# danshapero/sigma

Hardware: AMD Instinct MI355X
Metric: SpMV GB/s (achieved HBM) + CG iters/sec on 5-pt Laplacian, N=1e7 (higher is better)
Workload: dtype f64; 1 GPU; 5-point 2D Poisson CSR, 3162x3162 rows per GPU (rank 0: n=9998244, nnz=49978572), fp64 SpMV y=A*x; rows_per_gpu=9998244, nnz_per_gpu=49978572, parallelism=row-partition x1, matrix_resident_bytes_per_gpu=479920788, reference_layout_bytes_per_gpu=639735844, full=False

## Files before the change

sigma_amd/csrc/sgm_internal.hpp:

```cpp
#pragma once
#include <hip/hip_runtime.h>

#include <cstdarg>
#include <cstdint>
#include <cstdio>
#include <cstring>
#include <string>
#include <atomic>
#include <utility>
#include <vector>

#include "../../include/sigma_hip.h"

namespace sgm {

extern std::string g_err;
int fail(int code, const char *fmt, ...);

#define SGM_HIP(call)                                                              \
    do {                                                                           \
        hipError_t e__ = (call);                                                   \
        if (e__ != hipSuccess)                                                     \
            return sgm::fail(SGM_ERR_HIP, "%s:%d: %s -> %s", __FILE__, __LINE__,   \
                             #call, hipGetErrorString(e__));                       \
// ... 116 lines not shown

struct SliceSched { int32_t *tab = nullptr; int32_t lo = 0, hi = 0, grid = 0, iters = 0, band = 0; };

struct Part {
    MatOptions opt = g_opt.mat;
    int32_t n = 0;
    int32_t ncol_own = 0;
    int32_t n_halo = 0;
    int32_t int_lo = 0, int_hi = 0;
    int64_t nnz = 0;
    int64_t row_begin = 0;
    int32_t *rowptr = nullptr;
    int32_t *col = nullptr;
    double *val = nullptr;
    uint8_t *code = nullptr;
    int32_t *dict = nullptr;
    int32_t ndict = 0;
    int32_t dict_reach = 0;
    int32_t max_row = 0;
    double *sval = nullptr;
    uint32_t *scode = nullptr;
    int32_t *scol = nullptr;
    uint8_t *sbcode = nullptr;
    bool lean = false;
    double *sl_val = nullptr;
    int32_t *sl_col = nullptr;
    uint16_t *sl_perm = nullptr;
    int64_t *sl_off = nullptr;
    int64_t sl_total = 0;
    int32_t *sl_win0 = nullptr;
    int32_t sl_gs = 1;
    int32_t sl_span = 0;
    int32_t sw = 0;
    int32_t sched_period = 0;
    mutable SliceSched sched[3];
    mutable int nsched = 0;
    const int32_t *run_sched = nullptr;
    int32_t run_iters = 0;
    int32_t max_d = 0;
    int32_t *ecol = nullptr;
    double *eval = nullptr;
    int32_t *edeg = nullptr;
    uint8_t *ecode = nullptr;
    int32_t emdp = 0;
    int32_t *cb_perm = nullptr;
    double *cb_sval = nullptr;
    uint16_t *cb_lcol = nullptr;
    int32_t *cb_bstart = nullptr;
    uint16_t *cb_lpos = nullptr;
    void *cb_fdesc = nullptr;
    double *cb_P = nullptr;
    int32_t cb_cols = 0, cb_nb = 0, cb_R = 0, cb_ntiles = 0, cb_chunks = 0;
    int32_t cb_maxd = 0;
    int64_t cb_count = 0;
    double col_spread = -1.0;
    std::vector<HaloNbr> nbrs;
    double *xext = nullptr;
    int dot_grid_override = 0;
    int64_t xlen() const { return (int64_t)ncol_own + n_halo; }
};

}

namespace sgm { struct AlgPlan; void alg_plan_free(AlgPlan *p); void alg_plan_rows(const AlgPlan *p, int32_t out[2]); }

struct sgm_comm_s {
// ... 205 lines not shown
```

sigma_amd/csrc/sgm_layouts.hip:

```cpp
#include "sgm_spmv_select.hpp"

namespace sgm {

__global__ void k_dec1(int32_t *a, int64_t n)
{
    int64_t i = (int64_t)blockIdx.x * blockDim.x + threadIdx.x;
    const int64_t stride = (int64_t)gridDim.x * blockDim.x;
    for (; i < n; i += stride) a[i] -= 1;
}

__global__ void k_check_ptr1(const int32_t *__restrict__ ptr1, int64_t n, int64_t nnz, unsigned long long *bad)
{
    int64_t i = (int64_t)blockIdx.x * blockDim.x + threadIdx.x;
    const int64_t stride = (int64_t)gridDim.x * blockDim.x;
    for (; i <= n; i += stride) {
        const int32_t a = ptr1[i];
        bool ok = true;
        if (i == 0) ok = a == 1;
        if (i < n) ok = ok && ptr1[i + 1] >= a;
        else ok = ok && (int64_t)a - 1 == nnz;
        if (!ok) atomicMin(bad, (unsigned long long)i);
    }
}

// ... 227 lines not shown
        if (p.n > 0 && (mk_col || mk_val))
            hipLaunchKernelGGL(k_sell_unpack, dim3((unsigned)std::min<int64_t>((nch + 3) / 4, 65536)), dim3(256), 0, st, p.n,
                               (const int32_t *)p.rowptr, (const int64_t *)p.sl_off, (const uint16_t *)p.sl_perm, (const int32_t *)p.sl_col,
                               (const double *)p.sl_val, mk_col ? p.col : nullptr, mk_val ? p.val : nullptr);
        SGM_HIP(hipGetLastError());
        SGM_HIP(hipStreamSynchronize(st));
        return SGM_OK;
    }
    if (mk_code) { SGM_TRY(dalloc(&p.code, (size_t)nnz + 32)); SGM_HIP(hipMemsetAsync(p.code + nnz, 0, 32, st)); }
    if (p.n > 0)
        hipLaunchKernelGGL(k_sl_unpack, dim3((unsigned)std::min<int64_t>(((int64_t)p.n + 255) / 256, 4096)), dim3(256), 0, st, p.n, p.sw,
                           (const int32_t *)p.rowptr, (const uint32_t *)p.scode, (const int32_t *)p.dict, (const double *)p.sval,
                           mk_col ? p.col : nullptr, mk_val ? p.val : nullptr, mk_code ? p.code : nullptr);
    SGM_HIP(hipGetLastError());
    SGM_HIP(hipStreamSynchronize(st));
    return SGM_OK;
}
int lean_val_buffer(Part &p)
{
    if (!p.lean || p.val) return SGM_OK;
    SGM_TRY(dalloc(&p.val, (size_t)p.nnz + 2));
    SGM_HIP(hipMemsetAsync(p.val + p.nnz, 0, 2 * sizeof(double), g_rt.stream));
    return SGM_OK;
}
void csr_release_arrays(const Part &cp)
{
    Part &p = const_cast<Part &>(cp);
    if (!p.lean || !lean_applies(p)) return;
    (void)hipStreamSynchronize(g_rt.stream);
    dfree(p.val); dfree(p.col); dfree(p.code);
    p.val = nullptr; p.col = nullptr; p.code = nullptr;
}

int pack_sliced(Part &p)
{
    if (p.sl_val && p.n > 0) {
        const int64_t nch = (((int64_t)p.n + kSlRows - 1) / kSlRows) * (kSlRows / kSellChunk);
        hipLaunchKernelGGL(k_sell_fill, dim3((unsigned)std::min<int64_t>((nch + 3) / 4, 65536)), dim3(256), 0, g_rt.stream, p.n,
                           (const int32_t *)p.rowptr, (const int32_t *)nullptr, (const double *)p.val, (const int64_t *)p.sl_off,
                           (const uint16_t *)p.sl_perm, (int32_t *)nullptr, p.sl_val);
        SGM_HIP(hipGetLastError());
    }
    if ((!p.scode && !p.scol && !p.sbcode) || p.n == 0) return SGM_OK;
    const int64_t nsl = ((int64_t)p.n + kSlRows - 1) / kSlRows;
    if (p.ecol)
        hipLaunchKernelGGL(k_sl_pack_ell, dim3((unsigned)std::min<int64_t>(nsl, 65536)), dim3(256), 0, g_rt.stream, p.n, p.sw,
                           p.max_d, (const double *)p.eval, p.sval);
    else
        hipLaunchKernelGGL(k_sl_pack, dim3((unsigned)std::min<int64_t>(nsl, 65536)), dim3(256), 0, g_rt.stream, p.n, p.sw,
                           (const int32_t *)p.rowptr, (const double *)p.val, p.sval);
    SGM_HIP(hipGetLastError());
    return SGM_OK;
}

__global__ void k_fill32(int64_t n, int32_t *a, int32_t v)
{
    int64_t i = (int64_t)blockIdx.x * blockDim.x + threadIdx.x;
    const int64_t stride = (int64_t)gridDim.x * blockDim.x;
    for (; i < n; i += stride) a[i] = v;
}

constexpr int kDictSlots = 1024;
constexpr int32_t kDictEmpty = INT32_MIN;
__global__ __launch_bounds__(256) void k_dict_collect(int32_t n, const int32_t *__restrict__ rowptr, const int32_t *__restrict__ col,
                                                      int32_t *table, int *count, int *max_row)
{
    constexpr int kLocal = 512;
    __shared__ int32_t ltab[kLocal];
    __shared__ int lcount;
    for (int t = threadIdx.x; t < kLocal; t += 256) ltab[t] = kDictEmpty;
    if (threadIdx.x == 0) lcount = 0;
    __syncthreads();
    int mr = 0;
    int32_t mine[8];
#pragma unroll
    for (int t = 0; t < 8; ++t) mine[t] = kDictEmpty;
    int next = 0;
    for (int32_t i = blockIdx.x * blockDim.x + threadIdx.x; i < n; i += gridDim.x * blockDim.x) {
        const int32_t s0 = rowptr[i], e = rowptr[i + 1];
        mr = max(mr, e - s0);
        for (int32_t k = s0; k < e; ++k) {
            const int32_t off = col[k] - i;
            bool known = false;
#pragma unroll
            for (int t = 0; t < 8; ++t) known = known || mine[t] == off;
// ... 445 lines not shown
    *out = nullptr;
    if (!A || A->fmt != SGM_FMT_CSR || A->parts.size() != 1 || A->comm)
        return fail(SGM_ERR_UNSUPPORTED, "clone_csr_plain: single-GPU CSR matrices only");
    const Part &p = A->parts[0];
    SGM_TRY(csr_need_arrays(p));
    struct Release { const Part &p; ~Release() { csr_release_arrays(p); } } rel{p};
    sgm_mat C = new sgm_mat_s;
    C->fmt = SGM_FMT_CSR; C->nrow = A->nrow; C->ncol = A->ncol; C->nnz = A->nnz;
    C->parts.resize(1);
    Part &q = C->parts[0];
    q.opt.csr_offset_dict = 0; q.opt.csr_sliced = 0; q.opt.csr_sell = 0; q.opt.csr_lean = 0; q.opt.slice_sched = 0;
    q.n = p.n; q.ncol_own = p.ncol_own; q.n_halo = 0; q.nnz = p.nnz; q.max_row = p.max_row;
    hipStream_t st = g_rt.stream;
    int rc = dalloc(&q.rowptr, (size_t)p.n + 1);
    if (rc == SGM_OK) rc = dalloc(&q.col, (size_t)p.nnz + 4);
    if (rc == SGM_OK) rc = dalloc(&q.val, (size_t)p.nnz + 2);
    if (rc != SGM_OK) { sgm_mat_destroy(C); return rc; }
    (void)hipMemcpyAsync(q.rowptr, p.rowptr, ((size_t)p.n + 1) * 4, hipMemcpyDeviceToDevice, st);
    (void)hipMemsetAsync(q.col + p.nnz, 0, 16, st);
    (void)hipMemsetAsync(q.val + p.nnz, 0, 16, st);
    if (p.nnz) {
        (void)hipMemcpyAsync(q.col, p.col, (size_t)p.nnz * 4, hipMemcpyDeviceToDevice, st);
        (void)hipMemcpyAsync(q.val, p.val, (size_t)p.nnz * 8, hipMemcpyDeviceToDevice, st);
    }
    if (hipStreamSynchronize(st) != hipSuccess || hipGetLastError() != hipSuccess) { sgm_mat_destroy(C); return fail(SGM_ERR_HIP, "clone_csr_plain: copy failed"); }
    *out = C;
    return SGM_OK;
}

int rebuild_csr_formats(Part &p)
{
    SGM_TRY(csr_need_arrays(p));
    p.lean = false;
    dfree(p.code); dfree(p.dict); dfree(p.sval); dfree(p.scode); dfree(p.scol); dfree(p.sbcode);
    p.code = nullptr; p.dict = nullptr; p.sval = nullptr; p.scode = nullptr; p.scol = nullptr; p.sbcode = nullptr;
    free_sell(p);
    free_ell_colblock(p);
    p.ndict = 0; p.dict_reach = 0; p.sw = 0; p.max_row = 0; p.sched_period = 0;
    free_slice_sched(p);
    return build_offset_dict(p, nullptr, nullptr);
}
int rebuild_ell_formats(Part &p)
{
    dfree(p.ecode); dfree(p.dict); dfree(p.sval); dfree(p.scode);
    p.ecode = nullptr; p.dict = nullptr; p.dict_reach = 0; p.emdp = 0; p.sval = nullptr; p.scode = nullptr; p.sw = 0; p.sched_period = 0;
    free_slice_sched(p);
    SGM_TRY(build_ell_offset_dict(p));
    SGM_TRY(build_ell_colblock(p));
    return refresh_ell_colblock_values(p);
}
int sgm_invalidate_transpose(sgm_mat A)
{
    if (A->T) { sgm_mat_destroy(A->T); A->T = nullptr; }
    dfree(A->tperm);
    A->tperm = nullptr;
    A->t_stale = true;
    return SGM_OK;
}

void free_part(Part &p)
{
    dfree(p.rowptr); dfree(p.col); dfree(p.val); dfree(p.code); dfree(p.dict); dfree(p.sval); dfree(p.scode); dfree(p.scol); dfree(p.sbcode); dfree(p.ecol); dfree(p.eval); dfree(p.edeg); dfree(p.ecode); dfree(p.xext);
    for (auto &nb : p.nbrs) { dfree(nb.send_idx); dfree(nb.send_buf); }
    free_slice_sched(p);
    free_ell_colblock(p);
    free_sell(p);
    p = Part();
}

}
```

sigma_amd/csrc/sgm_mat.hip:

```cpp
#include "sgm_spmv_select.hpp"

namespace sgm {

struct Staged {
    double *dev = nullptr;
    bool owned = false;
    ~Staged() { if (owned) dfree(dev); }
};
int stage_in(Staged &s, const double *v, int64_t n, int where, bool copy)
{
    if (where == SGM_DEVICE && (reinterpret_cast<uintptr_t>(v) & 15) == 0) {
        s.dev = const_cast<double *>(v);
        return SGM_OK;
    }
    SGM_TRY(dalloc(&s.dev, (size_t)n));
    s.owned = true;
    if (copy)
        SGM_HIP(hipMemcpyAsync(s.dev, v, (size_t)n * 8,
                               where == SGM_HOST ? hipMemcpyHostToDevice : hipMemcpyDeviceToDevice,
                               g_rt.stream));
    return SGM_OK;
}
int stage_out(const Staged &s, double *v, int64_t n, int where)
{
// ... 361 lines not shown
    return SGM_OK;
}

int sgm_mat_set_option(sgm_mat A, const char *name, int value)
{
    SGM_TRY(require_init());
    if (!A || !name) return fail(SGM_ERR_BAD_ARG, "sgm_mat_set_option: null argument");
    int v = 0;
    SGM_TRY(normalise_option(name, value, &v));
    MatOptions probe;
    if (!mat_option_field(probe, name)) return fail(SGM_ERR_BAD_ARG, "sgm_mat_set_option: '%s' is not a matrix option", name);
    if (A->fmt == SGM_FMT_COMPOSITE) {
        for (sgm_mat_s *B : A->blocks)
            if (B) SGM_TRY(sgm_mat_set_option(B, name, value));
        return SGM_OK;
    }
    const bool cb_shape = !strcmp(name, "ell_colblock_cols") || !strcmp(name, "ell_colblock_rows");
    for (Part &p : A->parts) {
        int *f = mat_option_field(p.opt, name);
        const int old = *f;
        *f = v;
        if (old == v) continue;
        if ((p.ecol || (!p.lean && p.rowptr && p.col && p.val && p.n_halo == 0 && !p.sval && !p.sl_val)) &&
            (cb_shape || (!strcmp(name, "ell_colblock") && ((old != 0) != (v != 0) || v == 2 || old == 2)))) {
            SGM_TRY(build_ell_colblock(p));
            SGM_TRY(refresh_ell_colblock_values(p));
            SGM_HIP(hipStreamSynchronize(g_rt.stream));
        }
        if (!strcmp(name, "csr_lean") && !p.ecol) {
            if (v == 0) { SGM_TRY(csr_need_arrays(p)); p.lean = false; }
            else csr_go_lean(p);
        }
        if (!strcmp(name, "slice_sched")) free_slice_sched(p);
    }
    if (A->T) SGM_TRY(sgm_mat_set_option(A->T, name, value));
    return SGM_OK;
}

int sgm_mat_matvec(sgm_mat A, const double *x, double *y, int where)
{
    return matvec_impl(A, x, y, where, false);
}

int sgm_mat_matvec_add(sgm_mat A, const double *x, double *y, int where)
{
    return matvec_impl(A, x, y, where, true);
}

int sgm_composite_create(sgm_mat *out, int32_t nrb, int32_t ncb, const int32_t *row_ptr, const int32_t *col_ptr,
                         const sgm_mat *blocks)
{
    SGM_TRY(require_init());
    if (!out || nrb < 1 || ncb < 1 || !row_ptr || !col_ptr || !blocks)
        return fail(SGM_ERR_BAD_ARG, "sgm_composite_create: bad argument");
    sgm_mat A = new sgm_mat_s;
    A->fmt = SGM_FMT_COMPOSITE;
    for (int i = 0; i <= nrb; ++i) A->blk_row_ptr.push_back(row_ptr[i] - 1);
    for (int j = 0; j <= ncb; ++j) A->blk_col_ptr.push_back(col_ptr[j] - 1);
    A->nrow = A->blk_row_ptr[nrb];
    A->ncol = A->blk_col_ptr[ncb];
    A->blocks.assign(blocks, blocks + (size_t)nrb * ncb);
    sgm_comm comm = nullptr;
    bool any_local = false;
    for (int it = 0; it < nrb; ++it)
        for (int jt = 0; jt < ncb; ++jt) {
            sgm_mat C = A->blocks[(size_t)it * ncb + jt];
// ... 140 lines not shown
    else if (use_slicedb(p)) snprintf(name, len, "k_csr_slb<W=%d>", p.sw);
    else if (use_sliced32(p)) snprintf(name, len, "k_csr_sl32<W=%d>", p.sw);
    else if (use_sell(p)) snprintf(name, len, p.sl_win0 && p.opt.csr_xwindow ? "k_csr_sell<pad=%.3f,xw=%dx%d>" : "k_csr_sell<pad=%.3f>",
                                   p.nnz ? (double)p.sl_total / (double)p.nnz : 1.0, p.sl_span, p.sl_gs);
    else if (use_offset_dict(p)) snprintf(name, len, "k_csr_do<256,%d,CW=1>", do_tile_for(p));
    else if (use_row_owner(p)) snprintf(name, len, "k_csr_do<256,%d,CW=4>", do_tile_for(p));
    else if (use_row_lines(p)) snprintf(name, len, "k_csr_rl");
    else snprintf(name, len, "k_csr_spmv");
}
}
extern "C" {

int sgm_mat_kernel(sgm_mat A, char *buf, int len)
{
    if (!A || !buf || len < 1) return fail(SGM_ERR_BAD_ARG, "sgm_mat_kernel: bad argument");
    char name[64];
    if (A->fmt == SGM_FMT_COMPOSITE) snprintf(name, sizeof name, "composite");
    else part_kernel_name(A->parts[0], A->fmt, name, sizeof name);
    snprintf(buf, (size_t)len, "%s", name);
    return SGM_OK;
}

static int64_t part_resident_bytes(const Part &p)
{
    int64_t b = 0;
    const int64_t nsl = ((int64_t)p.n + kSlRows - 1) / kSlRows;
    if (p.rowptr) b += 4 * ((int64_t)p.n + 1);
    if (p.col) b += 4 * (p.nnz + 4);
    if (p.val) b += 8 * (p.nnz + 2);
    if (p.code) b += p.nnz + 16;
    if (p.dict) b += 4 * 256;
    if (p.sval) b += 8 * nsl * kSlRows * p.sw;
    if (p.scode) b += 4 * nsl * kSlRows;
    if (p.scol) b += 4 * nsl * kSlRows * p.sw;
    if (p.sbcode) b += nsl * kSlRows * ((p.sw + 7) / 8 * 8);
    if (p.sl_val) b += 12 * p.sl_total + 2 * nsl * kSlRows + 8 * (nsl * (kSlRows / kSellChunk) + 1);
    if (p.ecol) b += 4 * (int64_t)p.n * p.max_d;
    if (p.eval) b += 8 * (int64_t)p.n * p.max_d;
    if (p.edeg) b += 4 * (int64_t)p.n;
    if (p.ecode) b += (int64_t)p.n * p.emdp;
    if (p.xext) b += 8 * p.xlen();
    b += ell_colblock_resident_bytes(p);
    for (const auto &nb : p.nbrs) b += (int64_t)nb.send_count * (nb.send_buf ? 12 : 4);
    return b;
}
static int64_t part_matvec_bytes(const sgm_mat_s *A, const Part &p)
{
    const int64_t nsl = ((int64_t)p.n + kSlRows - 1) / kSlRows;
    int64_t m;
    if (A->fmt == SGM_FMT_ELL) {
        if (use_ell_colblock(p)) return ell_colblock_matvec_bytes(p);
        if (use_sliced_ell(p)) m = nsl * kSlRows * (8 * (int64_t)p.sw + 4);
        else if (p.ecode && p.opt.ell_offset_dict) m = (int64_t)p.n * (8 * (int64_t)p.max_d + p.emdp);
        else m = 12 * (int64_t)p.n * p.max_d;
    } else if (use_ell_colblock(p)) return ell_colblock_matvec_bytes(p);
    else if (use_sliced(p)) m = nsl * kSlRows * (8 * (int64_t)p.sw + 4);
    else if (use_slicedb(p)) m = nsl * kSlRows * (8 * (int64_t)p.sw + (p.sw + 7) / 8 * 8);
    else if (use_sliced32(p)) m = nsl * kSlRows * 12 * (int64_t)p.sw;
    else if (use_sell(p)) {
        m = 12 * p.sl_total + 2 * nsl * kSlRows + 8 * nsl * (kSlRows / kSellChunk);
        if (p.sl_win0 && p.opt.csr_xwindow)
            return m + ((nsl + p.sl_gs - 1) / p.sl_gs) * (8 * (int64_t)p.sl_span + 4) + 8 * (int64_t)p.n;
    }
    else if (use_offset_dict(p)) m = 9 * p.nnz + 4 * ((int64_t)p.n + 1);
    else m = 12 * p.nnz + 4 * ((int64_t)p.n + 1);
    return m + 8 * p.xlen() + 8 * (int64_t)p.n;
}

int sgm_mat_footprint(sgm_mat A, int64_t *resident_bytes, int64_t *matvec_bytes)
{
    if (!A) return fail(SGM_ERR_BAD_ARG, "sgm_mat_footprint: null matrix");
    int64_t res = 0, mv = 0;
    if (A->fmt == SGM_FMT_COMPOSITE) {
        for (sgm_mat C : A->blocks) {
            if (!C) continue;
            int64_t r = 0, m = 0;
            SGM_TRY(sgm_mat_footprint(C, &r, &m));
            mv += m + 8 * (int64_t)C->nrow;
        }
        mv += 8 * (int64_t)A->nrow;
    } else {
        for (const Part &p : A->parts) { res += part_resident_bytes(p); mv += part_matvec_bytes(A, p); }
        if (A->T) { int64_t r = 0; SGM_TRY(sgm_mat_footprint(A->T, &r, nullptr)); res += r + 4 * A->nnz; }
    }
    if (resident_bytes) *resident_bytes = res;
    if (matvec_bytes) *matvec_bytes = mv;
    return SGM_OK;
}

// ... 13 lines not shown
```

sigma_amd/csrc/sgm_runtime.hip:

```cpp
#include "sgm_internal.hpp"

#include <algorithm>

namespace sgm {

std::string g_err;
Runtime g_rt;
Options g_opt;
Heartbeat g_hb;
extern int g_force_collectives;

int fail(int code, const char *fmt, ...)
{
    char buf[1024];
    va_list ap;
    va_start(ap, fmt);
    vsnprintf(buf, sizeof buf, fmt, ap);
    va_end(ap);
    g_err = buf;
    return code;
}

bool trace_on()
{
// ... 60 lines not shown
    SGM_HIP(hipStreamSynchronize(st));
    return SGM_OK;
}

#define SGM_OPT(group, field) if (!strcmp(name, #field)) return &o.field;
int *mat_option_field(MatOptions &o, const char *name)
{
    SGM_OPT(mat, csr_offset_dict) SGM_OPT(mat, ell_offset_dict) SGM_OPT(mat, csr_row_owner) SGM_OPT(mat, csr_row_lines)
    SGM_OPT(mat, csr_sliced) SGM_OPT(mat, csr_sell) SGM_OPT(mat, csr_xwindow) SGM_OPT(mat, csr_lean) SGM_OPT(mat, ell_colblock) SGM_OPT(mat, ell_colblock_cols)
    SGM_OPT(mat, ell_colblock_rows) SGM_OPT(mat, slice_sched) SGM_OPT(mat, coloring_pass)
    return nullptr;
}
int *solver_option_field(SolverOptions &o, const char *name)
{
    SGM_OPT(solver, cg_small) SGM_OPT(solver, bicgstab_small) SGM_OPT(solver, krylov_graph) SGM_OPT(solver, dot_order)
    SGM_OPT(solver, gmres_cgs2) SGM_OPT(solver, dist_halo_fused) SGM_OPT(solver, coop_spin_limit) SGM_OPT(solver, cg_coop_variant)
    SGM_OPT(solver, reorder_solve)
    return nullptr;
}
int *pc_option_field(PcOptions &o, const char *name)
{
    SGM_OPT(pc, ildu_strips) SGM_OPT(pc, ildu_rows) SGM_OPT(pc, pipeline_spin_limit) SGM_OPT(pc, ildu_reorder)
    return nullptr;
}
#undef SGM_OPT

int normalise_option(const char *name, int value, int *out)
{
    int v = value;
    if (!strcmp(name, "ell_colblock_cols")) v = std::min(kEllcbMaxCols, std::max(2, value)) & ~1;
    else if (!strcmp(name, "ell_colblock_rows")) v = value == 512 ? 512 : value == 256 ? 256 : 0;
    else if (!strcmp(name, "ildu_reorder")) v = value != 0;
    else if (!strcmp(name, "csr_sell")) v = value < 0 ? 0 : value > 2 ? 2 : value;
    else if (!strcmp(name, "csr_lean") || !strcmp(name, "csr_xwindow")) v = value != 0;
    else if (!strcmp(name, "slice_sched")) v = value <= 0 ? 0 : value == 1 ? 1 : std::max(4, value);
    else if (!strcmp(name, "krylov_graph")) v = value <= 0 ? 0 : value == 1 ? 1 : std::max(16, (value + 15) / 16 * 16);
    else if (!strcmp(name, "cg_small")) v = std::max(0, value);
    else if (!strcmp(name, "dist_halo_fused") || !strcmp(name, "reorder_solve")) v = value < 0 ? 0 : value > 2 ? 2 : value;
    else if (!strcmp(name, "coop_spin_limit")) v = std::max(0, value);
    else if (!strcmp(name, "gmres_cgs2")) v = value != 0;
    else if (!strcmp(name, "cg_coop_variant")) {
        const int r = value & 15;
        if (value < 0 || value > 31 || (r != 0 && r != 1 && r != 2 && r != 4 && r != 8))
            return fail(SGM_ERR_BAD_ARG, "option cg_coop_variant: rows per thread 0 (by size), 1, 2, 4 or 8, + 16 = no one-XCD variant");
    }
    else if (!strcmp(name, "coloring_pass")) v = value < 0 ? 0 : value > 2 ? 2 : value;
    else if (!strcmp(name, "pipeline_spin_limit")) v = std::max(0, value);
    else if (!strcmp(name, "dot_order") && value != 0 && value != 1)
        return fail(SGM_ERR_BAD_ARG, "option dot_order is 0 (tree) or 1 (the reference's sequential order)");
    *out = v;
    return SGM_OK;
}

}

using namespace sgm;

extern "C" {

int sgm_init(int device)
{
    int count = 0;
    hipError_t e = hipGetDeviceCount(&count);
    if (e != hipSuccess || count <= 0)
        return fail(SGM_ERR_NO_DEVICE,
                    "sgm_init: no HIP device visible (%s); this library has no CPU path",
// ... 110 lines not shown
```

sigma_amd/csrc/sgm_spmv.hip:

```cpp
#include "sgm_spmv_select.hpp"
#include "sgm_plan_host.hpp"

namespace sgm {




__device__ inline int64_t rowblock_of(int it, int b, int grid, int64_t nrb = 0, int mode = 1)
{
    const int per = grid >> 3;
    if (mode == 2) {
        const int64_t chunk = (nrb + 7) / 8;
        const int64_t local = (int64_t)it * per + (b >> 3);
        return local < chunk ? (int64_t)(b & 7) * chunk + local : nrb;
    }
    return (int64_t)it * grid + (int64_t)(b & 7) * per + (b >> 3);
}


template <class T>
__device__ inline T ld_stream(const T *p, bool nt)
{
    return nt ? __builtin_nontemporal_load(p) : *p;
}
// ... 319 lines not shown
            while (k < kend) {
                const int cnt = min(kend - k, U);
                double xv[U], vv[U];
#pragma unroll
                for (int u = 0; u < U; ++u)
                    if (u < cnt) {
                        const int o = k + u - ts;
                        xv[u] = CW == 1 ? x[row + dl[cl[o]]] : x[(int32_t)cl4[o]];
                        vv[u] = vl[o];
                    }
#pragma unroll
                for (int u = 0; u < U; ++u)
                    if (u < cnt) z = z + vv[u] * xv[u];
                k += cnt;
            }
        }
        if (row < n) {
            const double yi = ADD ? (chain ? z : y0 + z) : 0.0 + z;
            __builtin_nontemporal_store(yi, y + row);
            if (DOT_W) dwy += w[row] * yi;
            if (DOT_YY) dyy += yi * yi;
        }
    }
    if (DOT_W) {
        const double t = block_sum<BLOCK>(dwy, red);
        if (tid == 0) part_wy[blockIdx.x] = t;
    }
    if (DOT_YY) {
        const double t = block_sum<BLOCK>(dyy, red);
        if (tid == 0) part_yy[blockIdx.x] = t;
    }
}

template <int W, bool ADD, bool DOT_W, bool DOT_YY>
__global__ __launch_bounds__(256) void k_csr_sl(
    int32_t n, const uint32_t *__restrict__ scode, const int32_t *__restrict__ dict,
    const double *__restrict__ sval, const double *__restrict__ x, double *__restrict__ y,
    const double *__restrict__ w, double *__restrict__ part_wy, double *__restrict__ part_yy,
    const int *__restrict__ flag_done, int gen, int remap, const int32_t *__restrict__ sched, int sched_iters)
{
    constexpr int BLOCK = 256;
    __shared__ int32_t dl[16];
    __shared__ double red[BLOCK / 64];
    const int st = flag_done ? *flag_done : 0;
    const int tid = threadIdx.x;
    const bool chain = (remap & 256) != 0;
    const int32_t dv = tid < 16 ? dict[tid] : 0;
    const int64_t nsl = ((int64_t)n + kSlRows - 1) / kSlRows;
    double dwy = 0.0, dyy = 0.0;

    int64_t first = blockIdx.x;
    if ((remap & 255) >= 3) {
        const int G = (remap & 255) == 3 ? 8 : (remap & 255) == 4 ? 2 : (remap & 255) == 6 ? 64 : (remap & 255) == 7 ? 128 : 32;
        const int xcd = blockIdx.x & 7, loc = blockIdx.x >> 3;
        first = (int64_t)(loc / G) * (8 * G) + xcd * G + loc % G;
    }
    int64_t sl = sched ? sched[blockIdx.x] : first;
    int sit = 0;
    u32x2 cw = {0xffffffffu, 0xffffffffu};
    f64x2 v[W];
    auto load_slice = [&](int64_t s_) {
        const int32_t row_ = (int32_t)(s_ * kSlRows) + 2 * tid;
        cw = __builtin_nontemporal_load(reinterpret_cast<const u32x2 *>(scode + row_));
        const f64x2 *vb = reinterpret_cast<const f64x2 *>(sval + s_ * (int64_t)(W * kSlRows)) + tid;
#pragma unroll
        for (int u = 0; u < W; ++u) v[u] = __builtin_nontemporal_load(vb + u * BLOCK);
    };
    bool have = sl >= 0 && sl < nsl;
    if (have) load_slice(sl);
    if (st && gen >= st) return;
    if (tid < 16) dl[tid] = dv;
    __syncthreads();
    while (have) {
        int64_t nxt = sl + gridDim.x;
        if (sched) { ++sit; nxt = sit < sched_iters ? sched[(int64_t)sit * gridDim.x + blockIdx.x] : -1; }
        const int32_t row = (int32_t)(sl * kSlRows) + 2 * tid;
        f64x2 y0 = {0.0, 0.0};
        if (ADD) {
            if (row + 1 < n) y0 = *reinterpret_cast<const f64x2 *>(y + row);
            else if (row < n) y0.x = y[row];
        }
        double xa[W], xb[W];
#pragma unroll
        for (int u = 0; u < W; ++u) {
            const uint32_t ca = (cw.x >> (4 * u)) & 15u, cb = (cw.y >> (4 * u)) & 15u;
            xa[u] = ca != 15u ? x[row + dl[ca]] : 0.0;
            xb[u] = cb != 15u ? x[row + 1 + dl[cb]] : 0.0;
        }
        f64x2 z;
        z.x = (ADD && chain) ? y0.x : 0.0;
        z.y = (ADD && chain) ? y0.y : 0.0;
#pragma unroll
        for (int u = 0; u < W; ++u) {
            if (((cw.x >> (4 * u)) & 15u) != 15u) z.x = z.x + v[u].x * xa[u];
            if (((cw.y >> (4 * u)) & 15u) != 15u) z.y = z.y + v[u].y * xb[u];
        }
        f64x2 yi;
        yi.x = ADD ? (chain ? z.x : y0.x + z.x) : 0.0 + z.x;
        yi.y = ADD ? (chain ? z.y : y0.y + z.y) : 0.0 + z.y;
        if (row + 1 < n) {
            __builtin_nontemporal_store(yi, reinterpret_cast<f64x2 *>(y + row));
            if (DOT_W) { const f64x2 wv = *reinterpret_cast<const f64x2 *>(w + row); dwy += wv.x * yi.x; dwy += wv.y * yi.y; }
            if (DOT_YY) { dyy += yi.x * yi.x; dyy += yi.y * yi.y; }
        } else if (row < n) {
            __builtin_nontemporal_store(yi.x, y + row);
            if (DOT_W) dwy += w[row] * yi.x;
            if (DOT_YY) dyy += yi.x * yi.x;
        }
        sl = nxt;
        have = sl >= 0 && sl < nsl;
        if (have) load_slice(sl);
    }
    if (DOT_W) {
        const double t = block_sum<BLOCK>(dwy, red);
        if (tid == 0) part_wy[blockIdx.x] = t;
    }
    if (DOT_YY) {
        const double t = block_sum<BLOCK>(dyy, red);
        if (tid == 0) part_yy[blockIdx.x] = t;
    }
}

template <bool ADD, bool DOT_W, bool DOT_YY, bool XW = false, int GS = 1>
__global__ __launch_bounds__(256 * GS) void k_csr_sell(
    int32_t n, const int64_t *__restrict__ off, const uint16_t *__restrict__ perm, const int32_t *__restrict__ scol,
    const double *__restrict__ sval, const double *__restrict__ x, double *__restrict__ y, const double *__restrict__ w,
    double *__restrict__ part_wy, double *__restrict__ part_yy, const int *__restrict__ flag_done, int gen, int remap,
    const int32_t *__restrict__ win0 = nullptr, int32_t span = 0, int32_t xlen = 0)
// ... 448 lines not shown
    const int tile = do_tile_for(p);
    const bool dict = use_offset_dict(p);
#define L(B, T, DW, DY)                                                                                 \
    do {                                                                                                \
        if (dict)                                                                                       \
            hipLaunchKernelGGL((k_csr_do<B, T, 1, ADD, DW, DY>), dim3(grid), dim3(B), 0, st, p.n, p.rowptr, \
                               p.code, p.dict, p.val, x, y, w, pwy, pyy, flag, gen, c.remap | g_launch_flags); \
        else                                                                                            \
            hipLaunchKernelGGL((k_csr_do<B, T, 4, ADD, DW, DY>), dim3(grid), dim3(B), 0, st, p.n, p.rowptr, \
                               reinterpret_cast<const uint8_t *>(p.col), p.dict, p.val, x, y, w, pwy, pyy, flag, \
                               gen, c.remap | g_launch_flags);                                          \
    } while (0)
#define LV(B, T)                                \
    if (c.block == B && tile == T) {            \
        if (w && pyy) L(B, T, true, true);      \
        else if (w) L(B, T, true, false);       \
        else if (pyy) L(B, T, false, true);     \
        else L(B, T, false, false);             \
        return;                                 \
    }
    SGM_DO_VARIANTS(LV)
#undef LV
#undef L
}

template <bool ADD>
static void launch_csr_sl(const Part &p, int grid, const double *x, double *y, const double *w,
                          double *pwy, double *pyy, const int *flag, int gen)
{
    const SpmvCfg &c = spmv_cfg();
    hipStream_t st = g_rt.stream;
    int mode = c.remap == 1 ? ((grid <= kMaxGrid / 2 || (int64_t)p.n < (int64_t)32768 * kSlRows) ? 5 : 0) : (c.remap >= 3 ? c.remap : 0);
    if (mode >= 3 && grid % (8 * (mode == 3 ? 8 : mode == 4 ? 2 : mode == 6 ? 64 : mode == 7 ? 128 : 32)) != 0) mode = 0;
#define L(WW, DW, DY)                                                                                   \
    hipLaunchKernelGGL((k_csr_sl<WW, ADD, DW, DY>), dim3(grid), dim3(256), 0, st, p.n, p.scode, p.dict, \
                       p.sval, x, y, w, pwy, pyy, flag, gen, mode | g_launch_flags, p.run_sched, p.run_iters)
#define LV(WW)                                \
    if (p.sw == WW) {                         \
        if (w && pyy) L(WW, true, true);      \
        else if (w) L(WW, true, false);       \
        else if (pyy) L(WW, false, true);     \
        else L(WW, false, false);             \
        return;                               \
    }
    SGM_SL_WIDTHS(LV)
#undef LV
#undef L
}

template <bool ADD>
static void launch_csr_sl32(const Part &p, int grid, const double *x, double *y, const double *w,
                            double *pwy, double *pyy, const int *flag, int gen)
{
    hipStream_t st = g_rt.stream;
    const SpmvCfg &c = spmv_cfg();
    int mode = c.remap == 1 ? ((grid <= kMaxGrid / 2 || (int64_t)p.n < (int64_t)32768 * kSlRows) ? 5 : 0) : (c.remap >= 3 ? c.remap : 0);
    if (mode >= 3 && grid % (8 * (mode == 3 ? 8 : mode == 4 ? 2 : mode == 6 ? 64 : mode == 7 ? 128 : 32)) != 0) mode = 0;
#define L(WW, DW, DY)                                                                                     \
    hipLaunchKernelGGL((k_csr_sl32<WW, ADD, DW, DY>), dim3(grid), dim3(256), 0, st, p.n, p.scol, p.sval, x, y, \
                       w, pwy, pyy, flag, gen, mode | g_launch_flags)
#define LV(WW)                                \
    if (p.sw == WW) {                         \
        if (w && pyy) L(WW, true, true);      \
        else if (w) L(WW, true, false);       \
        else if (pyy) L(WW, false, true);     \
        else L(WW, false, false);             \
        return;                               \
    }
    SGM_SL32_WIDTHS(LV)
#undef LV
#undef L
}

template <bool ADD>
static void launch_csr_sell(const Part &p, int grid, const double *x, double *y, const double *w,
                            double *pwy, double *pyy, const int *flag, int gen)
{
    hipStream_t st = g_rt.stream;
    const SpmvCfg &c = spmv_cfg();
// ... 57 lines not shown
static EllCfg &ell_cfg()
{
    static EllCfg c;
    static bool init = false;
    if (!init) {
        init = true;
        if (c.grid > kMaxGrid) c.grid = kMaxGrid;
    }
    return c;
}
int ell_grid(const Part &p)
{
    if (use_ell_colblock(p)) return ell_colblock_grid(p);
    if (use_sliced_ell(p)) {
        const int64_t nsl = ((int64_t)p.n + kSlRows - 1) / kSlRows;
        return (int)std::max<int64_t>(1, std::min<int64_t>(nsl, nsl >= 32768 ? kMaxGrid : kMaxGrid / 2));
    }
    int64_t g = ((int64_t)p.n + kBlock - 1) / kBlock;
    int64_t cap = ell_cfg().grid;
    if (p.ecode && p.opt.ell_offset_dict && p.emdp == 16) cap = std::min<int64_t>(cap, (int64_t)5 * g_rt.num_cu);
    return (int)std::max<int64_t>(1, std::min<int64_t>(g, cap));
}

template <bool ADD>
static void launch_ell(const Part &p, int grid, const double *x, double *y, const double *w,
                       double *pwy, double *pyy, const int *flag, int gen)
{
    if (use_ell_colblock(p)) {
        (void)launch_ell_colblock(p, grid, x, y, ADD, (g_launch_flags & 256) != 0, w, pwy, pyy, flag, gen);
        return;
    }
    if (use_sliced_ell(p)) {
        Part v;
        v.n = p.n; v.scode = p.scode; v.dict = p.dict; v.sval = p.sval; v.sw = p.sw;
        if (const SliceSched *ss = slice_sched(p, 0, p.n, grid)) { v.run_sched = ss->tab; v.run_iters = ss->iters; }
        launch_csr_sl<ADD>(v, grid, x, y, w, pwy, pyy, flag, gen);
        return;
    }
    hipStream_t st = g_rt.stream;
    const EllCfg &c = ell_cfg();
    if (p.ecode && p.opt.ell_offset_dict) {
#define LD(M, DW, DY)                                                                                   \
    hipLaunchKernelGGL((k_ell_do<M, ADD, DW, DY>), dim3(grid), dim3(kBlock), 0, st, p.n, p.max_d, p.ecode, \
                       p.dict, p.eval, x, y, w, pwy, pyy, flag, gen, g_launch_flags & 256)
#define LDV(M)                                   \
    {                                            \
        if (w && pyy) LD(M, true, true);         \
        else if (w) LD(M, true, false);          \
        else if (pyy) LD(M, false, true);        \
        else LD(M, false, false);                \
    }
        if (p.emdp == 4) LDV(4) else if (p.emdp == 8) LDV(8) else LDV(16)
#undef LDV
#undef LD
        return;
    }
#define L(UU, NTT, DW, DY)                                                                          \
    hipLaunchKernelGGL((k_ell_spmv<UU, NTT, ADD, DW, DY>), dim3(grid), dim3(kBlock), 0, st, p.n,     \
                       p.max_d, p.ecol, p.eval, x, y, w, pwy, pyy, flag, gen, g_launch_flags & 256)
#define LV(UU, NTT)                              \
    {                                            \
        if (w && pyy) L(UU, NTT, true, true);    \
        else if (w) L(UU, NTT, true, false);     \
        else if (pyy) L(UU, NTT, false, true);   \
        else L(UU, NTT, false, false);           \
    }
    if (c.u >= 16) { if (c.nt) LV(16, true) else LV(16, false) }
// ... 43 lines not shown
    for (int i = 0; i < p.nsched; ++i)
        if (p.sched[i].lo == lo && p.sched[i].hi == hi && p.sched[i].grid == grid) return p.sched[i].tab ? &p.sched[i] : nullptr;
    if (p.nsched >= 3) return nullptr;
    SliceSched &ss = p.sched[p.nsched++];
    ss.lo = lo; ss.hi = hi; ss.grid = grid; ss.tab = nullptr; ss.band = band;
    std::vector<int32_t> tab;
    int iters = 0;
    slice_sched_table(nsl, p.sched_period, grid, band, tab, iters);
    int32_t *d = nullptr;
    if (dalloc(&d, tab.size()) != SGM_OK) return nullptr;
    if (hipMemcpy(d, tab.data(), tab.size() * sizeof(int32_t), hipMemcpyHostToDevice) != hipSuccess) { dfree(d); return nullptr; }
    ss.tab = d; ss.iters = iters;
    return &ss;
}
void free_slice_sched(Part &p)
{
    for (int i = 0; i < p.nsched; ++i) { dfree(p.sched[i].tab); p.sched[i] = SliceSched(); }
    p.nsched = 0;
}

static void launch_range(sgm_mat A, const Part &p, const RowRange &r, const double *x, double *y, bool add,
                         const double *w, double *pwy, double *pyy, const int *flag_done, int gen)
{
    Part v;
    v.opt = p.opt;
    v.n = r.hi - r.lo;
    v.nnz = (int64_t)((double)p.nnz * v.n / (p.n > 0 ? p.n : 1));
    v.n_halo = p.n_halo; v.ncol_own = p.ncol_own;
    v.rowptr = p.rowptr + r.lo; v.col = p.col; v.val = p.val; v.code = p.code; v.dict = p.dict;
    v.max_row = p.max_row;
    const bool sliced = use_sliced(p), slicedb = !sliced && use_slicedb(p), sliced32 = !sliced && !slicedb && use_sliced32(p);
    if (sliced || slicedb)
        if (const SliceSched *ss = slice_sched(p, r.lo, r.hi, r.grid)) { v.run_sched = ss->tab; v.run_iters = ss->iters; }
    if (sliced) { v.sval = p.sval + (int64_t)r.lo * p.sw; v.scode = p.scode + r.lo; v.sw = p.sw; }
    if (slicedb) { v.sval = p.sval + (int64_t)r.lo * p.sw; v.sbcode = p.sbcode + (int64_t)r.lo * ((p.sw + 7) / 8 * 8); v.sw = p.sw; }
    if (sliced32) { v.sval = p.sval + (int64_t)r.lo * p.sw; v.scol = p.scol + (int64_t)r.lo * p.sw; v.sw = p.sw; }
    const bool sell = !sliced && !slicedb && !sliced32 && use_sell(p);
    if (sell) {
        v.sl_val = p.sl_val; v.sl_col = p.sl_col;
        v.sl_off = p.sl_off + r.lo / kSellChunk; v.sl_perm = p.sl_perm + r.lo;
        v.sl_gs = p.sl_gs;
        v.sl_win0 = p.sl_win0 ? p.sl_win0 + r.lo / (kSlRows * p.sl_gs) : nullptr; v.sl_span = p.sl_span;
    }
    const bool dict = use_offset_dict(p);
    const double *xs = dict ? x + r.lo : x;
    double *ys = y + r.lo;
    const double *ws = w ? w + r.lo : nullptr;
    double *pw = pwy ? pwy + r.part_off : nullptr, *py = pyy ? pyy + r.part_off : nullptr;
    if (sliced) {
        if (add) launch_csr_sl<true>(v, r.grid, xs, ys, ws, pw, py, flag_done, gen);
        else launch_csr_sl<false>(v, r.grid, xs, ys, ws, pw, py, flag_done, gen);
    } else if (slicedb) {
        if (add) launch_csr_slb<true>(v, r.grid, xs, ys, ws, pw, py, flag_done, gen);
        else launch_csr_slb<false>(v, r.grid, xs, ys, ws, pw, py, flag_done, gen);
    } else if (sliced32) {
        if (add) launch_csr_sl32<true>(v, r.grid, x, ys, ws, pw, py, flag_done, gen);
        else launch_csr_sl32<false>(v, r.grid, x, ys, ws, pw, py, flag_done, gen);
    } else if (sell) {
        if (add) launch_csr_sell<true>(v, r.grid, x, ys, ws, pw, py, flag_done, gen);
        else launch_csr_sell<false>(v, r.grid, x, ys, ws, pw, py, flag_done, gen);
    } else if (use_row_owner(p)) {
        if (add) launch_csr_do<true>(v, r.grid, xs, ys, ws, pw, py, flag_done, gen);
        else launch_csr_do<false>(v, r.grid, xs, ys, ws, pw, py, flag_done, gen);
    } else if (use_row_lines(p)) {
        if (add) launch_csr_rl<true>(v, r.grid, xs, ys, ws, pw, py, flag_done, gen);
        else launch_csr_rl<false>(v, r.grid, xs, ys, ws, pw, py, flag_done, gen);
    } else {
// ... 153 lines not shown
```

sigma_amd/csrc/sgm_spmv_select.hpp:

```cpp
#pragma once
#include "sgm_internal.hpp"

#include <type_traits>

#include <hipcub/hipcub.hpp>

#include <algorithm>
#include <cstdlib>
#include <string>
#include <vector>

namespace sgm {

typedef double f64x2 __attribute__((ext_vector_type(2)));
typedef int i32x2 __attribute__((ext_vector_type(2)));
typedef int i32x4 __attribute__((ext_vector_type(4)));
typedef uint32_t u32x2 __attribute__((ext_vector_type(2)));
typedef uint16_t u16x2 __attribute__((ext_vector_type(2)));
typedef unsigned int u32x4s __attribute__((ext_vector_type(4)));
#define SGM_SLB_WIDTHS(X) X(9) X(12) X(15) X(16) X(19) X(20) X(24) X(25) X(27) X(28) X(32)
#define SGM_SL_WIDTHS(X) X(3) X(5) X(7) X(8)
#define SGM_SL32_WIDTHS(X) X(3) X(5) X(7) X(8) X(12) X(16) X(20) X(24) X(28) X(32)
constexpr int kSlRows = 512;
constexpr int kSellChunk = 128;
constexpr int kSellSigma = 512;
static bool lean_sliced(const Part &p) { return p.scode && p.sval && p.dict && !p.ecol && !p.scol && !p.sbcode && p.sw <= 8; }
static bool lean_sell(const Part &p) { return p.sl_val && p.sl_col && !p.scode && !p.scol && !p.sbcode && !p.ecol; }
static bool lean_applies(const Part &p) { return p.opt.csr_lean && (lean_sliced(p) || lean_sell(p)); }


struct SpmvCfg { int block = 256, vpt = 2, nt = 1, maxgrid = 0, remap = 1, do_vpt = 0; };
static SpmvCfg &spmv_cfg()
{
    static SpmvCfg c;
    static bool init = false;
    if (!init) {
        init = true;
        if (c.maxgrid > kMaxGrid) c.maxgrid = kMaxGrid;
        if (c.block != 256 && c.block != 512 && c.block != 1024) c.block = 256;
        if (c.vpt != 2 && c.vpt != 4 && c.vpt != 8) c.vpt = 2;
        if (c.block == 1024 && c.vpt == 8) c.vpt = 4;
    }
    return c;
}

int resident_per_cu(bool dict, int block, int v, int cw = 4);
static const SliceSched *slice_sched(const Part &p, int32_t lo, int32_t hi, int grid);
void free_slice_sched(Part &p);
int ell_grid(const Part &p);
bool use_ell_colblock(const Part &p);
int ell_colblock_grid(const Part &p);
int build_ell_colblock(Part &p);
int refresh_ell_colblock_values(Part &p);
void free_ell_colblock(Part &p);
int launch_ell_colblock(const Part &p, int grid, const double *x, double *y, bool add, bool chain, const double *w,
                        double *pwy, double *pyy, const int *flag, int gen);
int64_t ell_colblock_resident_bytes(const Part &p);
// ... 49 lines not shown
    return (int)g;
}

struct RowRange { int32_t lo, hi; int grid, part_off; };
static int spmv_ranges(const Part &p, RowRange out[3], bool dots = true, bool whole = false)
{
    int nr = 0, off = 0;
    auto add = [&](int32_t lo, int32_t hi) {
        if (hi <= lo) return;
        out[nr] = RowRange{lo, hi, grid_for_rows(p, hi - lo, nr == 0 ? kMaxGrid / 4 : kMaxGrid / 8), off};
        off += out[nr].grid;
        ++nr;
    };
    if (p.n_halo == 0 || p.int_hi <= p.int_lo || whole) {
        if (any_sliced(p)) {
            out[0] = RowRange{0, p.n, grid_for_rows(p, p.n > 0 ? p.n : 1, kMaxGrid, dots), 0};
            return 1;
        }
        add(0, p.n > 0 ? p.n : 1);
        if (nr) out[0].hi = p.n;
        return nr;
    }
    add(p.int_lo, p.int_hi);
    add(0, p.int_lo);
    add(p.int_hi, p.n);
    return nr;
}


void free_part(Part &p);
void csr_go_lean(Part &p);
int lean_val_buffer(Part &p);
int pack_sliced(Part &p);
int build_ell_offset_dict(Part &p);
__global__ void k_ell_transpose(const int32_t *__restrict__ node, const double *__restrict__ val, int32_t *__restrict__ ecol,
                                double *__restrict__ eval, int32_t n, int32_t max_d, int32_t ncol = 0, unsigned long long *bad = nullptr);
}
```

Baseline: 6367 GB/s.

## Replace per-nonzero values with a per-code value table when codes map uniquely

After packing the sliced CSR format, a scan kernel checks whether every offset code always carries the same bit-exact value. If so, it builds a 16-entry value table, and the sliced SpMV kernel reads coefficients from shared memory instead of streaming sval. Where two adjacent rows share a code, the kernel also loads the pair of x values with one vector load. This removes most of the matrix value traffic for stencil-like matrices. The cost is an extra setup scan with a host synchronisation, a new template variant, and a much smaller modelled byte count per matvec.

```diff
diff --git a/sigma_amd/csrc/sgm_internal.hpp b/sigma_amd/csrc/sgm_internal.hpp
--- a/sigma_amd/csrc/sgm_internal.hpp
+++ b/sigma_amd/csrc/sgm_internal.hpp
@@ -172,6 +172,7 @@
     int32_t sl_gs = 1;
     int32_t sl_span = 0;
     int32_t sw = 0;
+    double *vtab = nullptr;
     int32_t sched_period = 0;
     mutable SliceSched sched[3];
     mutable int nsched = 0;
diff --git a/sigma_amd/csrc/sgm_layouts.hip b/sigma_amd/csrc/sgm_layouts.hip
--- a/sigma_amd/csrc/sgm_layouts.hip
+++ b/sigma_amd/csrc/sgm_layouts.hip
@@ -283,6 +283,78 @@
     p.val = nullptr; p.col = nullptr; p.code = nullptr;
 }
 
+__global__ __launch_bounds__(256) void k_sl_vtab_scan(int32_t n, int32_t W, const uint32_t *__restrict__ scode,
+                                                      const double *__restrict__ sval, unsigned long long *__restrict__ acc)
+{
+    __shared__ unsigned long long sand[16], sor[16];
+    __shared__ unsigned int sused;
+    if (threadIdx.x < 16) { sand[threadIdx.x] = ~0ull; sor[threadIdx.x] = 0ull; }
+    if (threadIdx.x == 0) sused = 0u;
+    __syncthreads();
+    unsigned int used = 0u;
+    const int64_t nsl = ((int64_t)n + kSlRows - 1) / kSlRows;
+    for (int64_t sl = blockIdx.x; sl < nsl; sl += gridDim.x)
+        for (int r = threadIdx.x; r < kSlRows; r += blockDim.x) {
+            const int64_t row = sl * kSlRows + r;
+            if (row >= n) break;
+            const uint32_t cw = scode[row];
+            const double *src = sval + sl * (int64_t)W * kSlRows + r;
+            for (int u = 0; u < W; ++u) {
+                const uint32_t c = (cw >> (4 * u)) & 15u;
+                if (c == 15u) continue;
+                const unsigned long long b = (unsigned long long)__double_as_longlong(src[(int64_t)u * kSlRows]);
+                atomicAnd(&sand[c], b);
+                atomicOr(&sor[c], b);
+                used |= 1u << c;
+            }
+        }
+    atomicOr(&sused, used);
+    __syncthreads();
+    const int t = threadIdx.x;
+    if (t < 16 && ((sused >> t) & 1u)) { atomicAnd(&acc[t], sand[t]); atomicOr(&acc[16 + t], sor[t]); }
+    if (t == 0 && sused) atomicOr(&acc[32], (unsigned long long)sused);
+}
+
+int find_value_table(Part &p)
+{
+    const int mode = p.opt.csr_sliced;
+    const bool want = p.scode && p.sval && !p.scol && !p.sbcode && !p.cb_sval && p.sw <= 8 && p.n > 0 && mode != 3 &&
+                      (mode == 2 || p.n >= (1 << 21));
+    if (!want) {
+        if (p.vtab) { SGM_HIP(hipStreamSynchronize(g_rt.stream)); dfree(p.vtab); p.vtab = nullptr; }
+        return SGM_OK;
+    }
+    double *buf = p.vtab;
+    p.vtab = nullptr;
+    if (!buf) SGM_TRY(dalloc(&buf, kVtabWords));
+    unsigned long long *acc = reinterpret_cast<unsigned long long *>(buf + 16);
+    SGM_HIP(hipMemsetAsync(acc, 0xff, 16 * 8, g_rt.stream));
+    SGM_HIP(hipMemsetAsync(acc + 16, 0, 17 * 8, g_rt.stream));
+    const int64_t nsl = ((int64_t)p.n + kSlRows - 1) / kSlRows;
+    hipLaunchKernelGGL(k_sl_vtab_scan, dim3((unsigned)std::min<int64_t>(nsl, 2048)), dim3(256), 0, g_rt.stream, p.n, p.sw,
+                       (const uint32_t *)p.scode, (const double *)p.sval, acc);
+    SGM_HIP(hipGetLastError());
+    unsigned long long h[33];
+    SGM_HIP(hipMemcpyAsync(h, acc, sizeof h, hipMemcpyDeviceToHost, g_rt.stream));
+    SGM_HIP(hipStreamSynchronize(g_rt.stream));
+    const uint32_t used = (uint32_t)h[32];
+    bool ok = used != 0;
+    unsigned long long tab[16] = {};
+    for (int c = 0; c < 15 && ok; ++c)
+        if ((used >> c) & 1u) { ok = h[c] == h[16 + c]; tab[c] = h[c]; }
+    if (ok) {
+        SGM_HIP(hipMemcpyAsync(buf, tab, sizeof tab, hipMemcpyHostToDevice, g_rt.stream));
+        SGM_HIP(hipStreamSynchronize(g_rt.stream));
+        p.vtab = buf;
+    } else {
+        dfree(buf);
+    }
+    if (trace_on())
+        fprintf(stderr, "[sgm] value table: %d rows, W=%d, %d codes used: %s\n", p.n, p.sw, __builtin_popcount(used),
+                ok ? "on (k_csr_sl reads no values)" : "off (a code carries more than one value)");
+    return SGM_OK;
+}
+
 int pack_sliced(Part &p)
 {
     if (p.sl_val && p.n > 0) {
@@ -301,7 +373,7 @@
         hipLaunchKernelGGL(k_sl_pack, dim3((unsigned)std::min<int64_t>(nsl, 65536)), dim3(256), 0, g_rt.stream, p.n, p.sw,
                            (const int32_t *)p.rowptr, (const double *)p.val, p.sval);
     SGM_HIP(hipGetLastError());
-    return SGM_OK;
+    return p.scode ? find_value_table(p) : SGM_OK;
 }
 
 __global__ void k_fill32(int64_t n, int32_t *a, int32_t v)
@@ -813,8 +885,8 @@
 {
     SGM_TRY(csr_need_arrays(p));
     p.lean = false;
-    dfree(p.code); dfree(p.dict); dfree(p.sval); dfree(p.scode); dfree(p.scol); dfree(p.sbcode);
-    p.code = nullptr; p.dict = nullptr; p.sval = nullptr; p.scode = nullptr; p.scol = nullptr; p.sbcode = nullptr;
+    dfree(p.code); dfree(p.dict); dfree(p.sval); dfree(p.scode); dfree(p.scol); dfree(p.sbcode); dfree(p.vtab);
+    p.code = nullptr; p.dict = nullptr; p.sval = nullptr; p.scode = nullptr; p.scol = nullptr; p.sbcode = nullptr; p.vtab = nullptr;
     free_sell(p);
     free_ell_colblock(p);
     p.ndict = 0; p.dict_reach = 0; p.sw = 0; p.max_row = 0; p.sched_period = 0;
@@ -823,8 +895,8 @@
 }
 int rebuild_ell_formats(Part &p)
 {
-    dfree(p.ecode); dfree(p.dict); dfree(p.sval); dfree(p.scode);
-    p.ecode = nullptr; p.dict = nullptr; p.dict_reach = 0; p.emdp = 0; p.sval = nullptr; p.scode = nullptr; p.sw = 0; p.sched_period = 0;
+    dfree(p.ecode); dfree(p.dict); dfree(p.sval); dfree(p.scode); dfree(p.vtab);
+    p.ecode = nullptr; p.dict = nullptr; p.dict_reach = 0; p.emdp = 0; p.sval = nullptr; p.scode = nullptr; p.vtab = nullptr; p.sw = 0; p.sched_period = 0;
     free_slice_sched(p);
     SGM_TRY(build_ell_offset_dict(p));
     SGM_TRY(build_ell_colblock(p));
@@ -841,7 +913,7 @@
 
 void free_part(Part &p)
 {
-    dfree(p.rowptr); dfree(p.col); dfree(p.val); dfree(p.code); dfree(p.dict); dfree(p.sval); dfree(p.scode); dfree(p.scol); dfree(p.sbcode); dfree(p.ecol); dfree(p.eval); dfree(p.edeg); dfree(p.ecode); dfree(p.xext);
+    dfree(p.rowptr); dfree(p.col); dfree(p.val); dfree(p.code); dfree(p.dict); dfree(p.sval); dfree(p.scode); dfree(p.scol); dfree(p.sbcode); dfree(p.ecol); dfree(p.eval); dfree(p.edeg); dfree(p.ecode); dfree(p.xext); dfree(p.vtab);
     for (auto &nb : p.nbrs) { dfree(nb.send_idx); dfree(nb.send_buf); }
     free_slice_sched(p);
     free_ell_colblock(p);
diff --git a/sigma_amd/csrc/sgm_mat.hip b/sigma_amd/csrc/sgm_mat.hip
--- a/sigma_amd/csrc/sgm_mat.hip
+++ b/sigma_amd/csrc/sgm_mat.hip
@@ -417,6 +417,7 @@
             else csr_go_lean(p);
         }
         if (!strcmp(name, "slice_sched")) free_slice_sched(p);
+        if (!strcmp(name, "csr_sliced") && p.scode) SGM_TRY(find_value_table(p));
     }
     if (A->T) SGM_TRY(sgm_mat_set_option(A->T, name, value));
     return SGM_OK;
@@ -623,6 +624,7 @@
     if (p.dict) b += 4 * 256;
     if (p.sval) b += 8 * nsl * kSlRows * p.sw;
     if (p.scode) b += 4 * nsl * kSlRows;
+    if (p.vtab) b += 8 * kVtabWords;
     if (p.scol) b += 4 * nsl * kSlRows * p.sw;
     if (p.sbcode) b += nsl * kSlRows * ((p.sw + 7) / 8 * 8);
     if (p.sl_val) b += 12 * p.sl_total + 2 * nsl * kSlRows + 8 * (nsl * (kSlRows / kSellChunk) + 1);
@@ -641,11 +643,11 @@
     int64_t m;
     if (A->fmt == SGM_FMT_ELL) {
         if (use_ell_colblock(p)) return ell_colblock_matvec_bytes(p);
-        if (use_sliced_ell(p)) m = nsl * kSlRows * (8 * (int64_t)p.sw + 4);
+        if (use_sliced_ell(p)) m = p.vtab ? 4 * nsl * kSlRows + 8 * 16 : nsl * kSlRows * (8 * (int64_t)p.sw + 4);
         else if (p.ecode && p.opt.ell_offset_dict) m = (int64_t)p.n * (8 * (int64_t)p.max_d + p.emdp);
         else m = 12 * (int64_t)p.n * p.max_d;
     } else if (use_ell_colblock(p)) return ell_colblock_matvec_bytes(p);
-    else if (use_sliced(p)) m = nsl * kSlRows * (8 * (int64_t)p.sw + 4);
+    else if (use_sliced(p)) m = p.vtab ? 4 * nsl * kSlRows + 8 * 16 : nsl * kSlRows * (8 * (int64_t)p.sw + 4);
     else if (use_slicedb(p)) m = nsl * kSlRows * (8 * (int64_t)p.sw + (p.sw + 7) / 8 * 8);
     else if (use_sliced32(p)) m = nsl * kSlRows * 12 * (int64_t)p.sw;
     else if (use_sell(p)) {
diff --git a/sigma_amd/csrc/sgm_runtime.hip b/sigma_amd/csrc/sgm_runtime.hip
--- a/sigma_amd/csrc/sgm_runtime.hip
+++ b/sigma_amd/csrc/sgm_runtime.hip
@@ -116,6 +116,7 @@
     else if (!strcmp(name, "ell_colblock_rows")) v = value == 512 ? 512 : value == 256 ? 256 : 0;
     else if (!strcmp(name, "ildu_reorder")) v = value != 0;
     else if (!strcmp(name, "csr_sell")) v = value < 0 ? 0 : value > 2 ? 2 : value;
+    else if (!strcmp(name, "csr_sliced")) v = value < 0 ? 0 : value > 3 ? 3 : value;
     else if (!strcmp(name, "csr_lean") || !strcmp(name, "csr_xwindow")) v = value != 0;
     else if (!strcmp(name, "slice_sched")) v = value <= 0 ? 0 : value == 1 ? 1 : std::max(4, value);
     else if (!strcmp(name, "krylov_graph")) v = value <= 0 ? 0 : value == 1 ? 1 : std::max(16, (value + 15) / 16 * 16);
diff --git a/sigma_amd/csrc/sgm_spmv.hip b/sigma_amd/csrc/sgm_spmv.hip
--- a/sigma_amd/csrc/sgm_spmv.hip
+++ b/sigma_amd/csrc/sgm_spmv.hip
@@ -375,20 +375,23 @@
     }
 }
 
-template <int W, bool ADD, bool DOT_W, bool DOT_YY>
+template <int W, bool ADD, bool DOT_W, bool DOT_YY, bool VT>
 __global__ __launch_bounds__(256) void k_csr_sl(
     int32_t n, const uint32_t *__restrict__ scode, const int32_t *__restrict__ dict,
     const double *__restrict__ sval, const double *__restrict__ x, double *__restrict__ y,
     const double *__restrict__ w, double *__restrict__ part_wy, double *__restrict__ part_yy,
-    const int *__restrict__ flag_done, int gen, int remap, const int32_t *__restrict__ sched, int sched_iters)
+    const int *__restrict__ flag_done, int gen, int remap, const int32_t *__restrict__ sched, int sched_iters,
+    const double *__restrict__ vtab)
 {
     constexpr int BLOCK = 256;
     __shared__ int32_t dl[16];
+    __shared__ double vl[VT ? 16 : 1];
     __shared__ double red[BLOCK / 64];
     const int st = flag_done ? *flag_done : 0;
     const int tid = threadIdx.x;
     const bool chain = (remap & 256) != 0;
     const int32_t dv = tid < 16 ? dict[tid] : 0;
+    const double tv = VT && tid < 16 ? vtab[tid] : 0.0;
     const int64_t nsl = ((int64_t)n + kSlRows - 1) / kSlRows;
     double dwy = 0.0, dyy = 0.0;
 
@@ -405,6 +408,7 @@
     auto load_slice = [&](int64_t s_) {
         const int32_t row_ = (int32_t)(s_ * kSlRows) + 2 * tid;
         cw = __builtin_nontemporal_load(reinterpret_cast<const u32x2 *>(scode + row_));
+        if (VT) return;
         const f64x2 *vb = reinterpret_cast<const f64x2 *>(sval + s_ * (int64_t)(W * kSlRows)) + tid;
 #pragma unroll
         for (int u = 0; u < W; ++u) v[u] = __builtin_nontemporal_load(vb + u * BLOCK);
@@ -412,7 +416,10 @@
     bool have = sl >= 0 && sl < nsl;
     if (have) load_slice(sl);
     if (st && gen >= st) return;
-    if (tid < 16) dl[tid] = dv;
+    if (tid < 16) {
+        dl[tid] = dv;
+        if (VT) vl[tid] = tv;
+    }
     __syncthreads();
     while (have) {
         int64_t nxt = sl + gridDim.x;
@@ -427,16 +434,24 @@
 #pragma unroll
         for (int u = 0; u < W; ++u) {
             const uint32_t ca = (cw.x >> (4 * u)) & 15u, cb = (cw.y >> (4 * u)) & 15u;
-            xa[u] = ca != 15u ? x[row + dl[ca]] : 0.0;
-            xb[u] = cb != 15u ? x[row + 1 + dl[cb]] : 0.0;
+            if (VT && ca == cb) {
+                f64x2u8 xp = {0.0, 0.0};
+                if (ca != 15u) xp = *reinterpret_cast<const f64x2u8 *>(x + row + dl[ca]);
+                xa[u] = xp.x;
+                xb[u] = xp.y;
+            } else {
+                xa[u] = ca != 15u ? x[row + dl[ca]] : 0.0;
+                xb[u] = cb != 15u ? x[row + 1 + dl[cb]] : 0.0;
+            }
         }
         f64x2 z;
         z.x = (ADD && chain) ? y0.x : 0.0;
         z.y = (ADD && chain) ? y0.y : 0.0;
 #pragma unroll
         for (int u = 0; u < W; ++u) {
-            if (((cw.x >> (4 * u)) & 15u) != 15u) z.x = z.x + v[u].x * xa[u];
-            if (((cw.y >> (4 * u)) & 15u) != 15u) z.y = z.y + v[u].y * xb[u];
+            const uint32_t ca = (cw.x >> (4 * u)) & 15u, cb = (cw.y >> (4 * u)) & 15u;
+            if (ca != 15u) z.x = z.x + (VT ? vl[ca] : v[u].x) * xa[u];
+            if (cb != 15u) z.y = z.y + (VT ? vl[cb] : v[u].y) * xb[u];
         }
         f64x2 yi;
         yi.x = ADD ? (chain ? z.x : y0.x + z.x) : 0.0 + z.x;
@@ -951,19 +966,26 @@
     hipStream_t st = g_rt.stream;
     int mode = c.remap == 1 ? ((grid <= kMaxGrid / 2 || (int64_t)p.n < (int64_t)32768 * kSlRows) ? 5 : 0) : (c.remap >= 3 ? c.remap : 0);
     if (mode >= 3 && grid % (8 * (mode == 3 ? 8 : mode == 4 ? 2 : mode == 6 ? 64 : mode == 7 ? 128 : 32)) != 0) mode = 0;
-#define L(WW, DW, DY)                                                                                   \
-    hipLaunchKernelGGL((k_csr_sl<WW, ADD, DW, DY>), dim3(grid), dim3(256), 0, st, p.n, p.scode, p.dict, \
-                       p.sval, x, y, w, pwy, pyy, flag, gen, mode | g_launch_flags, p.run_sched, p.run_iters)
+#define L(WW, DW, DY, VT)                                                                                   \
+    hipLaunchKernelGGL((k_csr_sl<WW, ADD, DW, DY, VT>), dim3(grid), dim3(256), 0, st, p.n, p.scode, p.dict,   \
+                       p.sval, x, y, w, pwy, pyy, flag, gen, mode | g_launch_flags, p.run_sched, p.run_iters, \
+                       (const double *)p.vtab)
+#define LT(WW, VT)                                \
+    {                                             \
+        if (w && pyy) L(WW, true, true, VT);      \
+        else if (w) L(WW, true, false, VT);       \
+        else if (pyy) L(WW, false, true, VT);     \
+        else L(WW, false, false, VT);             \
+    }
 #define LV(WW)                                \
     if (p.sw == WW) {                         \
-        if (w && pyy) L(WW, true, true);      \
-        else if (w) L(WW, true, false);       \
-        else if (pyy) L(WW, false, true);     \
-        else L(WW, false, false);             \
+        if (p.vtab) LT(WW, true)              \
+        else LT(WW, false)                    \
         return;                               \
     }
     SGM_SL_WIDTHS(LV)
 #undef LV
+#undef LT
 #undef L
 }
 
@@ -1087,7 +1109,7 @@
     }
     if (use_sliced_ell(p)) {
         Part v;
-        v.n = p.n; v.scode = p.scode; v.dict = p.dict; v.sval = p.sval; v.sw = p.sw;
+        v.n = p.n; v.scode = p.scode; v.dict = p.dict; v.sval = p.sval; v.sw = p.sw; v.vtab = p.vtab;
         if (const SliceSched *ss = slice_sched(p, 0, p.n, grid)) { v.run_sched = ss->tab; v.run_iters = ss->iters; }
         launch_csr_sl<ADD>(v, grid, x, y, w, pwy, pyy, flag, gen);
         return;
@@ -1197,7 +1219,7 @@
     const bool sliced = use_sliced(p), slicedb = !sliced && use_slicedb(p), sliced32 = !sliced && !slicedb && use_sliced32(p);
     if (sliced || slicedb)
         if (const SliceSched *ss = slice_sched(p, r.lo, r.hi, r.grid)) { v.run_sched = ss->tab; v.run_iters = ss->iters; }
-    if (sliced) { v.sval = p.sval + (int64_t)r.lo * p.sw; v.scode = p.scode + r.lo; v.sw = p.sw; }
+    if (sliced) { v.sval = p.sval + (int64_t)r.lo * p.sw; v.scode = p.scode + r.lo; v.sw = p.sw; v.vtab = p.vtab; }
     if (slicedb) { v.sval = p.sval + (int64_t)r.lo * p.sw; v.sbcode = p.sbcode + (int64_t)r.lo * ((p.sw + 7) / 8 * 8); v.sw = p.sw; }
     if (sliced32) { v.sval = p.sval + (int64_t)r.lo * p.sw; v.scol = p.scol + (int64_t)r.lo * p.sw; v.sw = p.sw; }
     const bool sell = !sliced && !slicedb && !sliced32 && use_sell(p);
diff --git a/sigma_amd/csrc/sgm_spmv_select.hpp b/sigma_amd/csrc/sgm_spmv_select.hpp
--- a/sigma_amd/csrc/sgm_spmv_select.hpp
+++ b/sigma_amd/csrc/sgm_spmv_select.hpp
@@ -13,6 +13,7 @@
 namespace sgm {
 
 typedef double f64x2 __attribute__((ext_vector_type(2)));
+typedef double f64x2u8 __attribute__((ext_vector_type(2), aligned(8)));
 typedef int i32x2 __attribute__((ext_vector_type(2)));
 typedef int i32x4 __attribute__((ext_vector_type(4)));
 typedef uint32_t u32x2 __attribute__((ext_vector_type(2)));
@@ -23,6 +24,7 @@
 #define SGM_SL32_WIDTHS(X) X(3) X(5) X(7) X(8) X(12) X(16) X(20) X(24) X(28) X(32)
 constexpr int kSlRows = 512;
 constexpr int kSellChunk = 128;
+constexpr int kVtabWords = 16 + 33;
 constexpr int kSellSigma = 512;
 static bool lean_sliced(const Part &p) { return p.scode && p.sval && p.dict && !p.ecol && !p.scol && !p.sbcode && p.sw <= 8; }
 static bool lean_sell(const Part &p) { return p.sl_val && p.sl_col && !p.scode && !p.scol && !p.sbcode && !p.ecol; }
@@ -138,6 +140,7 @@
 void csr_go_lean(Part &p);
 int lean_val_buffer(Part &p);
 int pack_sliced(Part &p);
+int find_value_table(Part &p);
 int build_ell_offset_dict(Part &p);
 __global__ void k_ell_transpose(const int32_t *__restrict__ node, const double *__restrict__ val, int32_t *__restrict__ ecol,
                                 double *__restrict__ eval, int32_t n, int32_t max_d, int32_t ncol = 0, unsigned long long *bad = nullptr);
```

Measured after the change: 4394 GB/s (median of 2 runs). 31.0% lower.
